# MuLabPKU/HD-PiSSA

Hardware: AMD Instinct MI355X
Metric: train tokens/sec (node) on the HD-PiSSA hot path, llama2-7b r16 (adapter probe fwd/bwd + Adam + dW aggregate + merge); dW merge+gather ms/step (higher is better)
Workload: dtype f32; 1 GPU; llama2-7b; model=llama2-7b, global_batch=16, seq_len=512, padding=per micro-batch to its longest sample (hp:190-201), micro_batches_per_rank=8, r_per_gpu=16, modules=224, exchange=gather, parallelism=dp1 (HD-PiSSA slices), x_layout=shared per projection group (q/k/v, gate/up)

## Files before the change

hd-pissa_amd/csrc/hdp_probe.hip:

```cpp
#include <chrono>
#include <cstdlib>
#include <cstring>
#include <mutex>
#include <vector>

#include "hdp_probe_int.h"

namespace hdp {

constexpr int kMaxGroup = 1024;
constexpr int kMaxSplit = 16;
constexpr int kP1Waves = 8;

static int p1_cols() {
  static const int v = [] { const char* e = getenv("HDP_P1_COLS"); return e ? atoi(e) : 128; }();
  return v;
}
static int p1_u() {
  static const int v = [] { const char* e = getenv("HDP_P1_U"); return e ? atoi(e) : 1; }();
  return v;
}
constexpr int kTC = 128;
constexpr int kNW = 256;

template <int CAP>
struct GroupArgsT {
  int n, rp, RB;
  int p1_pre[CAP + 1];
  int p2_pre[CAP + 1];
  int64_t p3_pre[CAP + 1];
  ProbeDesc d[CAP];
};
using GroupArgs = GroupArgsT<kMaxSplit>;
static_assert(sizeof(GroupArgs) <= 4096, "split-path kernel arguments must stay within 4 KB");

__device__ __forceinline__ int find_module(const int* pre, int n, int bid) {
  int m = 0;
  while (m + 1 < n && bid >= pre[m + 1]) ++m;
  return m;
}

template <bool F_RK>
__device__ __forceinline__ f32x4 load_f4(const float* F, int64_t K, int r, int j, int64_t k, int64_t k1, bool full) {
  f32x4 f;
  if (F_RK) {
    if (j < r && full) return *reinterpret_cast<const f32x4*>(F + (int64_t)j * K + k);
#pragma unroll
    for (int q = 0; q < 4; ++q) f[q] = (j < r && k + q < k1) ? F[(int64_t)j * K + k + q] : 0.f;
  } else {
#pragma unroll
    for (int q = 0; q < 4; ++q) f[q] = (j < r && k + q < k1) ? F[(k + q) * r + j] : 0.f;
  }
  return f;
}


template <int DT, int RB, int U, bool F_RK>
__device__ __forceinline__ void proj_wave(const void* Z, const float* F, int64_t T, int64_t K, int r, int64_t tb,
                                          int64_t k0, int64_t k1, int lane, float* tile, f32x4 (&acc)[RB]) {
// ... 308 lines not shown
}
__device__ __forceinline__ short bf16_bits(float v) { return (short)(__float_as_uint(v) >> 16); }
typedef __bf16 bf16x8 __attribute__((ext_vector_type(8)));
__device__ __forceinline__ void split8(const float (&v)[8], bf16x8& h, bf16x8& m, bf16x8& l) {
#pragma clang fp contract(off)
#pragma unroll
  for (int e = 0; e < 8; ++e) {
    const __bf16 a = (__bf16)v[e];
    const float r1 = v[e] - (float)a;
    const __bf16 b = (__bf16)r1;
    h[e] = a;
    m[e] = b;
    l[e] = (__bf16)(r1 - (float)b);
  }
}
__device__ __forceinline__ __bf16 as_bf16(float v) { return __builtin_bit_cast(__bf16, bf16_bits(v)); }
typedef uint32_t u32x4s __attribute__((ext_vector_type(4)));
__device__ __forceinline__ void split8p(const float (&v)[8], bf16x8& h, bf16x8& m, bf16x8& l) {
#pragma clang fp contract(off)
  u32x4s H, M, L;
#pragma unroll
  for (int e = 0; e < 4; ++e) {
    const float a0 = v[2 * e], a1 = v[2 * e + 1];
    const uint32_t ph = cvt_pk_bf16(a0, a1);
    const float r0 = a0 - __uint_as_float(ph << 16), r1 = a1 - __uint_as_float(ph & 0xffff0000u);
    const uint32_t pm = cvt_pk_bf16(r0, r1);
    const float s0 = r0 - __uint_as_float(pm << 16), s1 = r1 - __uint_as_float(pm & 0xffff0000u);
    H[e] = ph;
    M[e] = pm;
    L[e] = cvt_pk_bf16(s0, s1);
  }
  h = __builtin_bit_cast(bf16x8, H);
  m = __builtin_bit_cast(bf16x8, M);
  l = __builtin_bit_cast(bf16x8, L);
}
__device__ __forceinline__ f32x4 mfma_x6(const bf16x8 (&x)[3], const bf16x8 (&y)[3], f32x4 c) {
  c = __builtin_amdgcn_mfma_f32_16x16x32_bf16(x[1], y[1], c, 0, 0, 0);
  c = __builtin_amdgcn_mfma_f32_16x16x32_bf16(x[2], y[0], c, 0, 0, 0);
  c = __builtin_amdgcn_mfma_f32_16x16x32_bf16(x[0], y[2], c, 0, 0, 0);
  c = __builtin_amdgcn_mfma_f32_16x16x32_bf16(x[1], y[0], c, 0, 0, 0);
  c = __builtin_amdgcn_mfma_f32_16x16x32_bf16(x[0], y[1], c, 0, 0, 0);
  return __builtin_amdgcn_mfma_f32_16x16x32_bf16(x[0], y[0], c, 0, 0, 0);
}
__device__ __forceinline__ f32x4 mfma32(bf16x8 a, bf16x8 b, f32x4 c) {
  return __builtin_amdgcn_mfma_f32_16x16x32_bf16(a, b, c, 0, 0, 0);
}
__device__ __forceinline__ f32x4 mfma_bf16(bf16x4 a, bf16x4 b, f32x4 c) {
  return __builtin_amdgcn_mfma_f32_16x16x16bf16_1k(a, b, c, 0, 0, 0);
}

constexpr int kSwRedBufs = 4;
template <int RB, bool FUSE = false>
constexpr int sw_nbuf() { return FUSE ? 3 : RB >= 4 ? 2 : kSwRedBufs; }
#ifndef HDP_BF_SETS
#define HDP_BF_SETS 3
#endif
constexpr int kBfSets = HDP_BF_SETS;
enum { kSwProj = 1, kSwOuter = 2 };

template <int RB>
__device__ __forceinline__ void sw_store_g(const SweepDesc& d, const f32x4 (&acc2)[RB][4], int64_t col, int g,
                                           bool vec) {
#pragma clang fp contract(off)
  const float sc = d.scale;
  const int r = d.r;
  const int64_t N = d.N;
  if (!d.part_t) {
#pragma unroll
    for (int b = 0; b < RB; ++b)
#pragma unroll
      for (int reg = 0; reg < 4; ++reg) {
        const int j = 16 * b + 4 * g + reg;
        if (j >= r) continue;
        float* p = d.g + (int64_t)j * N + col;
        const f32x4 v{sc * acc2[b][0][reg], sc * acc2[b][1][reg], sc * acc2[b][2][reg], sc * acc2[b][3][reg]};
        if (vec) {
          gst4(p, d.acc ? gld4(p) + v : v);
        } else {
#pragma unroll
          for (int q = 0; q < 4; ++q)
            if (col + q < N) gst1(p + q, d.acc ? gld1(p + q) + v[q] : v[q]);
        }
      }
  } else {
    const bool v4 = (d.ldb & 3) == 0 && (reinterpret_cast<uintptr_t>(d.g) & 15) == 0;
#pragma unroll
    for (int b = 0; b < RB; ++b)
#pragma unroll
      for (int q = 0; q < 4; ++q) {
        if (col + q >= N) continue;
        const int j0 = 16 * b + 4 * g;
        float* p = d.g + (col + q) * d.ldb + j0;
        const f32x4 v = sc * acc2[b][q];
        if (v4 && j0 + 3 < r) {
          gst4(p, d.acc ? gld4(p) + v : v);
        } else {
#pragma unroll
          for (int reg = 0; reg < 4; ++reg)
            if (j0 + reg < r) gst1(p + reg, d.acc ? gld1(p + reg) + v[reg] : v[reg]);
        }
      }
  }
}

__device__ __forceinline__ void sw_store_g_fuse(const SweepDesc& d, const f32x4 (&acc2)[kSwMaxBlk][4], int64_t col,
                                                int g, bool vec) {
// ... 6 lines not shown
      const float sc = d.sc[b];
      const int acc = d.accb[b];
#pragma unroll
      for (int reg = 0; reg < 4; ++reg) {
        const int j = 4 * g + reg;
        if (j >= d.rbr[b]) continue;
        float* p = d.gb[b] + (int64_t)j * N + col;
        const f32x4 v{sc * acc2[b][0][reg], sc * acc2[b][1][reg], sc * acc2[b][2][reg], sc * acc2[b][3][reg]};
        if (vec) {
          gst4(p, acc ? gld4(p) + v : v);
        } else {
#pragma unroll
          for (int q = 0; q < 4; ++q)
            if (col + q < N) gst1(p + q, acc ? gld1(p + q) + v[q] : v[q]);
        }
      }
    }
  } else {
    const float sc = d.scale;
    const int r = d.r;
    const bool v4 = (d.ldb & 3) == 0 && (reinterpret_cast<uintptr_t>(d.g) & 15) == 0;
#pragma unroll
    for (int b = 0; b < kSwMaxBlk; ++b) {
      if (b >= d.nb) break;
#pragma unroll
      for (int q = 0; q < 4; ++q) {
        if (col + q >= N) continue;
        const int j0 = 16 * b + 4 * g;
        float* p = d.g + (col + q) * d.ldb + j0;
        const f32x4 v = sc * acc2[b][q];
        if (v4 && j0 + 3 < r) {
          gst4(p, d.acc ? gld4(p) + v : v);
        } else {
#pragma unroll
          for (int reg = 0; reg < 4; ++reg)
            if (j0 + reg < r) gst1(p + reg, d.acc ? gld1(p + reg) + v[reg] : v[reg]);
        }
      }
    }
  }
}

struct SweepArgs {
  int n, G;
  int spin;
  int64_t U;
  int* err;
  int* errd;
  const SweepDesc* d;
  const int* wst;
  const int* bnd;
};

template <int DT, int RB, int MODE, bool VEC, int OCC, bool FUSE, bool K32>
__device__ __forceinline__ void sweep_segment(const SweepDesc& d, int ct, int s0, int n, int64_t i0, int piece,
                                              const SweepArgs& sa, float* tile, float* red, int* flags, int wave,
                                              int lane) {
  constexpr bool PROJ = (MODE & kSwProj) != 0, OUTER = (MODE & kSwOuter) != 0;
  constexpr int rp = 16 * RB, r4 = rp / 4, ES = DT == HDP_F32 ? 4 : 2;
  const int li = lane & 15, g = lane >> 4;
  const int64_t T = d.T, N = d.N;
  const int64_t c = (int64_t)ct * kSwC + 64 * wave;
  const int64_t col = c + 4 * li;
  const int64_t colc = VEC ? (col < N ? col : N - 4) : col;
  const char* Zb = reinterpret_cast<const char*>(d.Z);

  constexpr bool SPLIT_F = DT == HDP_BF16 && MODE == kSwProj;
  constexpr bool X6 = K32 && DT == HDP_F32;
  constexpr bool K32P = K32 && MODE == kSwProj, K32O = K32 && MODE == kSwOuter;
  constexpr bool DL = K32P && DT == HDP_BF16 && !X6 && VEC;
  const int64_t cdl0 = c + 8 * g < N ? c + 8 * g : N - 8, cdl1 = c + 32 + 8 * g < N ? c + 32 + 8 * g : N - 8;
  f32x4 f[K32P ? 1 : 4][RB];
  bf16x4 fs[K32P ? 1 : 4][RB][3];
  bf16x8 fs8[K32P ? 2 : 1][RB][3];
  if constexpr (K32P) {
#pragma unroll
    for (int ch = 0; ch < 2; ++ch)
#pragma unroll
      for (int b = 0; b < RB; ++b) {
        const int j = 16 * b + li;
        const int64_t k = c + 32 * ch + 8 * g;
        float v[8];
#pragma unroll
        for (int e = 0; e < 8; ++e) v[e] = 0.f;
        const float* Fp = nullptr;
        int rows = d.r;
        if constexpr (FUSE) {
          Fp = b < d.nb ? d.Fb[b] : nullptr;
          rows = b < d.nb ? d.rbr[b] : 0;
        }
        const bool ok = FUSE ? (Fp != nullptr && li < rows) : (j < d.r);
        if (ok) {
          if (FUSE) Fp += (int64_t)li * N;
          if ((FUSE || d.f_rk) && N % 4 == 0 && k + 7 < N) {
            const float* P = FUSE ? Fp : d.F + (int64_t)j * N;
            const f32x4 a = gld4(P + k), bq = gld4(P + k + 4);
#pragma unroll
            for (int e = 0; e < 4; ++e) {
              v[e] = a[e];
              v[4 + e] = bq[e];
            }
          } else {
#pragma unroll
            for (int e = 0; e < 8; ++e)
              if (k + e < N)
                v[e] = FUSE ? gld1(Fp + k + e)
                            : d.f_rk ? gld1(d.F + (int64_t)j * N + k + e) : gld1(d.F + (k + e) * d.r + j);
          }
        }
        split8(v, fs8[ch][b][0], fs8[ch][b][1], fs8[ch][b][2]);
#pragma unroll
        for (int t = 0; t < 3; ++t) asm volatile("" : "+v"(fs8[ch][b][t]));
      }
  }
  if constexpr (PROJ && !K32P) {
#pragma unroll
    for (int s = 0; s < 4; ++s)
#pragma unroll
      for (int b = 0; b < RB; ++b) {
        const int j = 16 * b + li;
        const int64_t k = c + 16 * s + 4 * g;
        f32x4 v{0.f, 0.f, 0.f, 0.f};
        if constexpr (FUSE) {
          if (b < d.nb && li < d.rbr[b]) {
            const float* Fp = d.Fb[b] + (int64_t)li * N;
            if (N % 4 == 0 && k + 3 < N) {
              v = gld4(Fp + k);
            } else {
#pragma unroll
              for (int q = 0; q < 4; ++q)
                if (k + q < N) v[q] = gld1(Fp + k + q);
            }
          }
        } else if (j < d.r) {
          if (d.f_rk && N % 4 == 0 && k + 3 < N) {
            v = gld4(d.F + (int64_t)j * N + k);
          } else {
#pragma unroll
            for (int q = 0; q < 4; ++q)
              if (k + q < N) v[q] = d.f_rk ? gld1(d.F + (int64_t)j * N + k + q) : gld1(d.F + (k + q) * d.r + j);
          }
        }
        f[s][b] = v;
      }
    if constexpr (SPLIT_F) {
#pragma unroll
      for (int s = 0; s < 4; ++s)
#pragma unroll
        for (int b = 0; b < RB; ++b) {
          split3(f[s][b], fs[s][b][0], fs[s][b][1], fs[s][b][2]);
#pragma unroll
          for (int t = 0; t < 3; ++t) asm volatile("" : "+v"(fs[s][b][t]));
        }
    } else {
#pragma unroll
      for (int s = 0; s < 4; ++s)
#pragma unroll
        for (int b = 0; b < RB; ++b) asm volatile("" : "+v"(f[s][b]));
    }
  }
  bool hs_broken = false;
  f32x4 acc2[OUTER ? RB : 1][4];
#pragma unroll
  for (int b = 0; b < (OUTER ? RB : 1); ++b)
#pragma unroll
    for (int q = 0; q < 4; ++q) acc2[b][q] = f32x4{0.f, 0.f, 0.f, 0.f};

  constexpr bool DIST = PROJ && !FUSE && RB >= 4;
  int pend_i = -1, pend_s = 0;
  bool pend_tail = false;
  auto wait_ge = [&](const int* p, int target) {
    if (hs_broken) return;
    int it = 0;
    while (sa.spin < 0 || __hip_atomic_load(p, __ATOMIC_RELAXED, __HIP_MEMORY_SCOPE_WORKGROUP) < target) {
      if (it++ >= sa.spin) {
        hs_broken = true;
        if (lane == 0) {
          __hip_atomic_store(sa.err, 1, __ATOMIC_RELAXED, __HIP_MEMORY_SCOPE_SYSTEM);
          __hip_atomic_store(sa.errd, 1, __ATOMIC_RELAXED, __HIP_MEMORY_SCOPE_AGENT);
        }
        break;
      }
      __builtin_amdgcn_s_sleep(1);
    }
    asm volatile("" ::: "memory");
  };
  auto reduce_slice = [&](int pi, int ps, bool ptail) {
    if constexpr (DIST) {
      constexpr int NB = sw_nbuf<RB, FUSE>();
      const int pb = pi % NB, pr = pi / NB;
      wait_ge(flags + pb, kSwWaves * (pr + 1));
      const float* rs = red + pb * kSwWaves * 16 * rp;
      const int idx = 2 * lane;
      if (idx < 2 * rp) {
        const int row = 2 * wave + idx / rp, j = idx % rp;
        typedef float f32x2s __attribute__((ext_vector_type(2)));
        f32x2s acc{0.f, 0.f};
#pragma unroll
        for (int ww = 0; ww < kSwWaves; ++ww) acc += *reinterpret_cast<const f32x2s*>(rs + (ww * 16 + row) * rp + j);
        const int64_t t = 16 * (int64_t)ps + row;
        if (!ptail || t < T) *reinterpret_cast<HDP_GLOBAL f32x2s*>(gptr(d.slab_out + ((int64_t)ct * T + t) * rp + j)) = acc;
      }
      asm volatile("s_waitcnt lgkmcnt(0)" ::: "memory");
      if (lane == 0) (void)__hip_atomic_fetch_add(flags + NB + pb, 1, __ATOMIC_RELAXED, __HIP_MEMORY_SCOPE_WORKGROUP);
    }
  };

  auto compute = [&](const f32x4 (&z)[4], const float (&y)[4][RB], int s, int64_t i, bool tail) {
    if constexpr (OUTER) {
      if constexpr (DT == HDP_BF16) {
#pragma unroll
        for (int b = 0; b < RB; ++b) {
          if (FUSE && b >= d.nb) break;
          f32x4 yv;
#pragma unroll
          for (int p = 0; p < 4; ++p) yv[p] = (!tail || 16 * (int64_t)s + 4 * p + g < T) ? y[p][b] : 0.f;
          bf16x4 yh, ym, yl;
          split3(yv, yh, ym, yl);
#pragma unroll
          for (int q = 0; q < 4; ++q) {
            const bf16x4 zb{bf16_bits(z[0][q]), bf16_bits(z[1][q]), bf16_bits(z[2][q]), bf16_bits(z[3][q])};
            acc2[b][q] = mfma_bf16(yl, zb, acc2[b][q]);
            acc2[b][q] = mfma_bf16(ym, zb, acc2[b][q]);
            acc2[b][q] = mfma_bf16(yh, zb, acc2[b][q]);
          }
        }
      } else {
#pragma unroll
        for (int p = 0; p < 4; ++p) {
          const bool rok = !tail || 16 * (int64_t)s + 4 * p + g < T;
#pragma unroll
          for (int b = 0; b < RB; ++b) {
            if (FUSE && b >= d.nb) break;
            const float yv = rok ? y[p][b] : 0.f;
#pragma unroll
            for (int q = 0; q < 4; ++q) acc2[b][q] = __builtin_amdgcn_mfma_f32_16x16x4f32(yv, z[p][q], acc2[b][q], 0, 0, 0);
          }
        }
      }
    }
    if constexpr (PROJ) {
#pragma unroll
      for (int p = 0; p < (DL ? 0 : 4); ++p) *reinterpret_cast<f32x4*>(tile + (4 * p + g) * kTileLd + 4 * li) = z[p];
      f32x4 a0[RB], a1[RB];
#pragma unroll
      for (int b = 0; b < RB; ++b) a0[b] = a1[b] = f32x4{0.f, 0.f, 0.f, 0.f};
      if constexpr (K32P) {
#pragma unroll
        for (int ch = 0; ch < 2; ++ch) {
          f32x4 lo4{0.f, 0.f, 0.f, 0.f}, hi4{0.f, 0.f, 0.f, 0.f};
          if constexpr (!DL) {
            lo4 = *reinterpret_cast<const f32x4*>(tile + li * kTileLd + 32 * ch + 8 * g);
            hi4 = *reinterpret_cast<const f32x4*>(tile + li * kTileLd + 32 * ch + 8 * g + 4);
          }
          if constexpr (X6) {
            const float zv[8] = {lo4[0], lo4[1], lo4[2], lo4[3], hi4[0], hi4[1], hi4[2], hi4[3]};
            bf16x8 zs[3];
            split8p(zv, zs[0], zs[1], zs[2]);
#pragma unroll
            for (int b = 0; b < RB; ++b) {
              if (FUSE && b >= d.nb) break;
              f32x4& a = ch ? a1[b] : a0[b];
              a = mfma_x6(zs, fs8[ch][b], a);
            }
          } else {
            bf16x8 zb;
            if constexpr (DL) {
              zb = __builtin_bit_cast(bf16x8, z[ch]);
            } else {
#pragma unroll
              for (int e = 0; e < 4; ++e) {
                zb[e] = as_bf16(lo4[e]);
                zb[4 + e] = as_bf16(hi4[e]);
              }
            }
#pragma unroll
            for (int b = 0; b < RB; ++b) {
              if (FUSE && b >= d.nb) break;
              f32x4& a = ch ? a1[b] : a0[b];
              a = mfma32(zb, fs8[ch][b][2], a);
              a = mfma32(zb, fs8[ch][b][1], a);
              a = mfma32(zb, fs8[ch][b][0], a);
            }
          }
        }
      }
#pragma unroll
      for (int ss = 0; ss < (K32P ? 0 : 4); ++ss) {
        const f32x4 zf = *reinterpret_cast<const f32x4*>(tile + li * kTileLd + 16 * ss + 4 * g);
        if constexpr (SPLIT_F) {
          const bf16x4 zb{bf16_bits(zf[0]), bf16_bits(zf[1]), bf16_bits(zf[2]), bf16_bits(zf[3])};
#pragma unroll
          for (int b = 0; b < RB; ++b) {
            if (FUSE && b >= d.nb) break;
            f32x4& a = (ss & 1) ? a1[b] : a0[b];
            a = mfma_bf16(zb, fs[ss][b][2], a);
            a = mfma_bf16(zb, fs[ss][b][1], a);
            a = mfma_bf16(zb, fs[ss][b][0], a);
          }
        } else {
#pragma unroll
          for (int b = 0; b < RB; ++b) {
            if (FUSE && b >= d.nb) break;
#pragma unroll
            for (int q = 0; q < 4; ++q) {
              if (ss & 1) a1[b] = __builtin_amdgcn_mfma_f32_16x16x4f32(zf[q], f[ss][b][q], a1[b], 0, 0, 0);
              else a0[b] = __builtin_amdgcn_mfma_f32_16x16x4f32(zf[q], f[ss][b][q], a0[b], 0, 0, 0);
            }
          }
        }
      }
      HDP_MFMA_FENCE();
      constexpr int NBUF = sw_nbuf<RB, FUSE>();
      const int bsel = (int)(i % NBUF);
      const int round = (int)(i / NBUF);
      int* arrive = flags + bsel;
      int* done = flags + NBUF + bsel;
      if constexpr (DIST) {
        if (round > 0) wait_ge(done, kSwWaves * round);
        float* rb = red + (bsel * kSwWaves + wave) * 16 * rp;
#pragma unroll
        for (int b = 0; b < RB; ++b)
#pragma unroll
          for (int reg = 0; reg < 4; ++reg) rb[(4 * g + reg) * rp + 16 * b + li] = a0[b][reg] + a1[b][reg];
        asm volatile("s_waitcnt lgkmcnt(0)" ::: "memory");
        if (lane == 0) (void)__hip_atomic_fetch_add(arrive, 1, __ATOMIC_RELAXED, __HIP_MEMORY_SCOPE_WORKGROUP);
        if (pend_i >= 0) reduce_slice(pend_i, pend_s, pend_tail);
        pend_i = i;
        pend_s = s;
        pend_tail = tail;
      } else {
        if (round > 0 && !hs_broken) {
          int it = 0;
          while (sa.spin < 0 || __hip_atomic_load(done, __ATOMIC_RELAXED, __HIP_MEMORY_SCOPE_WORKGROUP) < round) {
            if (it++ >= sa.spin) {
              hs_broken = true;
              if (lane == 0) {
                __hip_atomic_store(sa.err, 1, __ATOMIC_RELAXED, __HIP_MEMORY_SCOPE_SYSTEM);
                __hip_atomic_store(sa.errd, 1, __ATOMIC_RELAXED, __HIP_MEMORY_SCOPE_AGENT);
              }
              break;
            }
            __builtin_amdgcn_s_sleep(1);
          }
          asm volatile("" ::: "memory");
        }
        float* rb = red + (bsel * kSwWaves + wave) * 16 * rp;
#pragma unroll
        for (int b = 0; b < RB; ++b) {
          if (FUSE && b >= d.nb) break;
#pragma unroll
          for (int reg = 0; reg < 4; ++reg) rb[(4 * g + reg) * rp + 16 * b + li] = a0[b][reg] + a1[b][reg];
        }
        asm volatile("s_waitcnt lgkmcnt(0)" ::: "memory");
        int old = 0;
        if (lane == 0) old = __hip_atomic_fetch_add(arrive, 1, __ATOMIC_RELAXED, __HIP_MEMORY_SCOPE_WORKGROUP);
        old = __builtin_amdgcn_readfirstlane(old);
        if (old == kSwWaves - 1) {
          asm volatile("s_waitcnt lgkmcnt(0)" ::: "memory");
          const float* rs = red + bsel * kSwWaves * 16 * rp;
          if constexpr (FUSE) {
#pragma unroll
            for (int b = 0; b < RB; ++b) {
              if (b >= d.nb) break;
              const int row = lane >> 2, jj = (lane & 3) * 4;
              f32x4 acc{0.f, 0.f, 0.f, 0.f};
#pragma unroll
              for (int ww = 0; ww < kSwWaves; ++ww)
                acc += *reinterpret_cast<const f32x4*>(rs + (ww * 16 + row) * rp + 16 * b + jj);
              const int64_t t = 16 * (int64_t)s + row;
              if (!tail || t < T) gst4(d.slab_b[b] + ((int64_t)ct * T + t) * d.rpm + jj, acc);
            }
          } else {
#pragma unroll
            for (int e0 = 0; e0 < 16 * r4; e0 += 64) {
              const int e = e0 + lane, row = e / r4, j = (e % r4) * 4;
              f32x4 acc{0.f, 0.f, 0.f, 0.f};
#pragma unroll
              for (int ww = 0; ww < kSwWaves; ++ww) acc += *reinterpret_cast<const f32x4*>(rs + (ww * 16 + row) * rp + j);
              const int64_t t = 16 * (int64_t)s + row;
              if (!tail || t < T) gst4(d.slab_out + ((int64_t)ct * T + t) * rp + j, acc);
            }
          }
          asm volatile("s_waitcnt lgkmcnt(0)" ::: "memory");
          if (lane == 0) {
            __hip_atomic_store(arrive, 0, __ATOMIC_RELAXED, __HIP_MEMORY_SCOPE_WORKGROUP);
            __hip_atomic_store(done, round + 1, __ATOMIC_RELAXED, __HIP_MEMORY_SCOPE_WORKGROUP);
          }
        }
      }
    }
  };

  auto pair = [&](const f32x4 (&zA)[4], const float (&yA)[4][RB], const f32x4 (&zB)[4], const float (&yB)[4][RB],
                  int s, bool vB, bool tail) {
    if constexpr (K32O && X6) {
      bf16x8 zs[4][3];
#pragma unroll
      for (int q = 0; q < 4; ++q) {
        const float zv[8] = {zA[0][q], zA[1][q], zA[2][q], zA[3][q],
                             vB ? zB[0][q] : 0.f, vB ? zB[1][q] : 0.f, vB ? zB[2][q] : 0.f, vB ? zB[3][q] : 0.f};
        split8p(zv, zs[q][0], zs[q][1], zs[q][2]);
      }
#pragma unroll
      for (int b = 0; b < RB; ++b) {
        if (FUSE && b >= d.nb) break;
        float yv[8];
#pragma unroll
        for (int p = 0; p < 4; ++p) {
          yv[p] = (!tail || 16 * (int64_t)s + 4 * p + g < T) ? yA[p][b] : 0.f;
          yv[4 + p] = vB ? yB[p][b] : 0.f;
        }
        bf16x8 ys[3];
        split8p(yv, ys[0], ys[1], ys[2]);
#pragma unroll
        for (int q = 0; q < 4; ++q) acc2[b][q] = mfma_x6(ys, zs[q], acc2[b][q]);
      }
    } else if constexpr (K32O) {
      bf16x8 zq[4];
#pragma unroll
      for (int q = 0; q < 4; ++q)
#pragma unroll
        for (int p = 0; p < 4; ++p) {
          zq[q][p] = as_bf16(zA[p][q]);
          zq[q][4 + p] = as_bf16(zB[p][q]);
        }
#pragma unroll
      for (int b = 0; b < RB; ++b) {
        if (FUSE && b >= d.nb) break;
        float yv[8];
#pragma unroll
        for (int p = 0; p < 4; ++p) {
          yv[p] = (!tail || 16 * (int64_t)s + 4 * p + g < T) ? yA[p][b] : 0.f;
          yv[4 + p] = vB ? yB[p][b] : 0.f;
        }
        bf16x8 yh, ym, yl;
        split8(yv, yh, ym, yl);
#pragma unroll
        for (int q = 0; q < 4; ++q) {
          acc2[b][q] = mfma32(yl, zq[q], acc2[b][q]);
          acc2[b][q] = mfma32(ym, zq[q], acc2[b][q]);
          acc2[b][q] = mfma32(yh, zq[q], acc2[b][q]);
        }
      }
    }
  };

  const int full_end = (int)min((int64_t)(s0 + n), T / 16);
  const int nfull = full_end > s0 ? full_end - s0 : 0;
  if (nfull > 0) {
    int64_t zo[4];
    int yo[4];
#pragma unroll
    for (int p = 0; p < 4; ++p) {
      zo[p] = ((16 * (int64_t)s0 + 4 * p + g) * N + colc) * ES;
      yo[p] = (16 * s0 + 4 * p + g) * d.yrs + li * d.yls;
    }
    const int64_t zstep = 16 * N * ES;
    int64_t zd = (16 * (int64_t)s0 + li) * N * ES;
    int lk = 0;
    auto load = [&](f32x4 (&z)[4], float (&y)[4][RB]) {
      __builtin_amdgcn_sched_barrier(0);
      if constexpr (DL) {
        typedef uint32_t u32x4d __attribute__((ext_vector_type(4)));
        z[0] = __builtin_bit_cast(f32x4, *reinterpret_cast<const HDP_GLOBAL u32x4d*>(gptr(Zb + zd + cdl0 * ES)));
        z[1] = __builtin_bit_cast(f32x4, *reinterpret_cast<const HDP_GLOBAL u32x4d*>(gptr(Zb + zd + cdl1 * ES)));
      }
#pragma unroll
      for (int p = 0; p < (DL ? 0 : 4); ++p) {
        if constexpr (VEC) {
          if constexpr (DT == HDP_F32)
            z[p] = load4_nt<DT>(Zb + zo[p], 0);
          else
            z[p] = load4<DT>(Zb + zo[p], 0);
        } else {
          const int64_t rowoff = zo[p] / ES - colc;
#pragma unroll
          for (int q = 0; q < 4; ++q) z[p][q] = load1<DT>(d.Z, rowoff + (col + q < N ? col + q : N - 1));
        }
        if constexpr (OUTER) {
          if constexpr (RB == 4) {
            const f32x4 v = gld4(d.y_in + yo[p]);
#pragma unroll
            for (int b = 0; b < RB; ++b) y[p][b] = v[b];
          } else if constexpr (RB == 2) {
            typedef float f32x2 __attribute__((ext_vector_type(2)));
            const f32x2 v = *reinterpret_cast<const HDP_GLOBAL f32x2*>(gptr(d.y_in + yo[p]));
            y[p][0] = v[0];
            y[p][1] = v[1];
          } else {
#pragma unroll
            for (int b = 0; b < RB; ++b) y[p][b] = gld1(d.y_in + yo[p] + b);
          }
        }
      }
      __builtin_amdgcn_sched_barrier(0);
      if (lk + 1 < nfull) {
        ++lk;
        zd += zstep;
#pragma unroll
        for (int p = 0; p < 4; ++p) {
          zo[p] += zstep;
// ... 22 lines not shown
      for (int j = 0; j + 1 < NS; ++j) load(zz[j], yy[j]);
      for (int k = 0; k < nfull; k += NS) {
#pragma unroll
        for (int j = 0; j < NS; ++j) {
          load(zz[(j + NS - 1) % NS], yy[(j + NS - 1) % NS]);
          if (j == 0 || k + j < nfull) compute(zz[j], yy[j], s0 + k + j, i0 + k + j, false);
        }
      }
    } else {
      f32x4 z0[4], z1[4];
      float y0[4][RB], y1[4][RB];
      load(z0, y0);
      for (int k = 0; k < nfull; k += 2) {
        load(z1, y1);
        compute(z0, y0, s0 + k, i0 + k, false);
        load(z0, y0);
        if (k + 1 < nfull) compute(z1, y1, s0 + k + 1, i0 + k + 1, false);
      }
    }
  }
  if (nfull < n) {
    const int s = s0 + nfull;
    f32x4 z[4];
    float y[4][RB];
    if constexpr (DL) {
      typedef uint32_t u32x4d __attribute__((ext_vector_type(4)));
      int64_t row = 16 * (int64_t)s + li;
      row = row < T ? row : T - 1;
      z[0] = __builtin_bit_cast(f32x4, *reinterpret_cast<const HDP_GLOBAL u32x4d*>(gptr(Zb + (row * N + cdl0) * ES)));
      z[1] = __builtin_bit_cast(f32x4, *reinterpret_cast<const HDP_GLOBAL u32x4d*>(gptr(Zb + (row * N + cdl1) * ES)));
    }
#pragma unroll
    for (int p = 0; p < (DL ? 0 : 4); ++p) {
      int64_t row = 16 * (int64_t)s + 4 * p + g;
      row = row < T ? row : T - 1;
      if constexpr (VEC) {
        z[p] = load4<DT>(d.Z, row * N + colc);
      } else {
#pragma unroll
        for (int q = 0; q < 4; ++q) z[p][q] = load1<DT>(d.Z, row * N + (col + q < N ? col + q : N - 1));
      }
      if constexpr (OUTER) {
#pragma unroll
        for (int b = 0; b < RB; ++b) y[p][b] = gld1(d.y_in + row * d.yrs + li * d.yls + b);
      }
    }
    if constexpr (K32O)
      pair(z, y, z, y, s, false, true);
    else
      compute(z, y, s, i0 + nfull, true);
  }
  if constexpr (DIST) {
    if (pend_i >= 0) reduce_slice(pend_i, pend_s, pend_tail);
  }
  if constexpr (OUTER) {
    HDP_MFMA_FENCE();
    if (s0 == 0 && n == d.S) {
      if constexpr (FUSE) {
        if (col < N) sw_store_g_fuse(d, acc2, col, g, VEC);
      } else {
        if (col < N) sw_store_g<RB>(d, acc2, col, g, VEC);
      }
    } else if (FUSE && col < N) {
      const int64_t pofs = ((int64_t)ct * d.kmax + piece) * d.rpm * kSwC;
#pragma unroll
      for (int b = 0; b < RB; ++b) {
        if (b >= d.nb) break;
        float* base = d.part_b[b] + pofs;
        if (!d.part_t) {
#pragma unroll
          for (int reg = 0; reg < 4; ++reg)
            gst4(base + (4 * g + reg) * kSwC + 64 * wave + 4 * li,
                 f32x4{acc2[b][0][reg], acc2[b][1][reg], acc2[b][2][reg], acc2[b][3][reg]});
        } else {
#pragma unroll
          for (int q = 0; q < 4; ++q) gst4(base + (64 * wave + 4 * li + q) * d.rpm + 4 * g, acc2[b][q]);
        }
      }
    } else if (col < N) {
      float* base = d.part + ((int64_t)ct * d.kmax + piece) * rp * kSwC;
      if (!d.part_t) {
#pragma unroll
        for (int b = 0; b < RB; ++b)
#pragma unroll
          for (int reg = 0; reg < 4; ++reg)
            gst4(base + (16 * b + 4 * g + reg) * kSwC + 64 * wave + 4 * li,
                 f32x4{acc2[b][0][reg], acc2[b][1][reg], acc2[b][2][reg], acc2[b][3][reg]});
      } else {
#pragma unroll
        for (int b = 0; b < RB; ++b)
#pragma unroll
          for (int q = 0; q < 4; ++q)
            gst4(base + (64 * wave + 4 * li + q) * rp + 16 * b + 4 * g, acc2[b][q]);
      }
    }
  }
}

template <int DT, int RB, int MODE, bool VEC, int OCC, bool FUSE = false, bool K32 = false>
__global__ __launch_bounds__(512, OCC == 2 ? 4 : 2) void probe_sweep_kernel(SweepArgs sa) {
  extern __shared__ __attribute__((aligned(16))) float lds[];
  const int w = blockIdx.x;
  const int64_t nsteps = sa.bnd[w + 1] - sa.bnd[w];
  if (nsteps <= 0) return;
  const int lane = threadIdx.x & 63, wave = threadIdx.x >> 6;
  float* tile = lds + wave * 16 * kTileLd;
  float* red = lds + kSwWaves * 16 * kTileLd;
  int* flags = reinterpret_cast<int*>(red + sw_nbuf<RB, FUSE>() * kSwWaves * 16 * 16 * RB);
  if constexpr ((MODE & kSwProj) != 0) {
    if (threadIdx.x < 2 * sw_nbuf<RB, FUSE>()) flags[threadIdx.x] = 0;
    __syncthreads();
  }
  int m = sa.wst[4 * w], ct = sa.wst[4 * w + 1], s = sa.wst[4 * w + 2];
  int piece = sa.wst[4 * w + 3];
  for (int64_t done = 0; done < nsteps;) {
    const SweepDesc d = sa.d[m];
    const int n = (int)min((int64_t)(d.S - s), nsteps - done);
    sweep_segment<DT, RB, MODE, VEC, OCC, FUSE, K32>(d, ct, s, n, done, piece, sa, tile, red, flags, wave, lane);
    done += n;
    s = 0;
    piece = 0;
    if (++ct == d.nct) {
      ct = 0;
      ++m;
    }
  }
}

struct YReduceArgs {
  int n, rp;
  const YRedDesc* d;
};

__global__ __launch_bounds__(256) void probe_yreduce_kernel(YReduceArgs ya) {
  const YRedDesc d = ya.d[blockIdx.y];
  const int64_t f = (int64_t)blockIdx.x * 256 + threadIdx.x;
  const int64_t step4 = d.T * ya.rp / 4;
  if (f >= step4) return;
  const f32x4* src = reinterpret_cast<const f32x4*>(d.slab) + f;
  f32x4 acc{0.f, 0.f, 0.f, 0.f};
  for (int c0 = 0; c0 < d.nct; c0 += 8) {
    f32x4 v[8];
#pragma unroll
    for (int u = 0; u < 8; ++u) v[u] = c0 + u < d.nct ? gld4(reinterpret_cast<const float*>(src + (c0 + u) * step4)) : f32x4{0.f, 0.f, 0.f, 0.f};
#pragma unroll
    for (int u = 0; u < 8; ++u) acc += v[u];
  }
  const int rp = ya.rp;
  const int64_t e = 4 * f, t = e / rp;
  const int j0 = (int)(e % rp), b = j0 / 16, li0 = j0 % 16;
  float* dst = d.y + t * d.ys + b;
#pragma unroll
  for (int k = 0; k < 4; ++k) gst1(dst + (li0 + k) * d.sl, acc[k]);
}

struct SwFinishArgs {
  int n, rp;
  const FinDesc* d;
  const int* jobs;
  int bx;
};

template <int V>
__global__ __launch_bounds__(256) void probe_sweep_finish_kernel(SwFinishArgs fa) {
#pragma clang fp contract(off)
  typedef float vec __attribute__((ext_vector_type(V)));
  const int job = blockIdx.x / fa.bx;
  const FinDesc& dm = fa.d[fa.jobs[4 * job]];
  const int code = fa.jobs[4 * job + 1], ct = code >> 1;
  const bool sideA = (code & 1) == 0;
  const int r = dm.r;
// ... 192 lines not shown
    switch (p1_u()) {
      case 1: hipLaunchKernelGGL((probe_proj_kernel<DT, RB, 1>), g1, b1, lds1(1), st, ga); break;
      case 3: hipLaunchKernelGGL((probe_proj_kernel<DT, RB, 3>), g1, b1, lds1(3), st, ga); break;
      default: hipLaunchKernelGGL((probe_proj_kernel<DT, RB, 2>), g1, b1, lds1(2), st, ga); break;
    }
  }
  }
  HDP_CHECK_LAUNCH();
  {
    KTimer kt(K_PROBE_P2, st, w.xg, w.fl_x + w.fl_g);
    hipLaunchKernelGGL((probe_outer_kernel<DT, RB>), dim3(ga.p2_pre[ga.n]), dim3(512),
                       (size_t)(kTC * rp > 4096 ? kTC * rp : 4096) * sizeof(float), st, ga);
  }
  HDP_CHECK_LAUNCH();
  const int64_t tot = ga.p3_pre[ga.n];
  const int blocks = (int)min((int64_t)4096, (tot + 255) / 256);
  bool v4 = true;
  int64_t per = 1;
  for (int i = 0; i < ga.n; ++i) {
    const ProbeDesc& d = ga.d[i];
    v4 = v4 && d.r % 4 == 0 && d.in % 4 == 0 && (reinterpret_cast<uintptr_t>(d.gA) & 15) == 0 &&
         (reinterpret_cast<uintptr_t>(d.gB) & 15) == 0 && (reinterpret_cast<uintptr_t>(d.partA) & 15) == 0 &&
         (reinterpret_cast<uintptr_t>(d.partB) & 15) == 0;
    const int64_t e = ((int64_t)d.r * (d.in + d.out) + 1023) / 1024;
    per = e > per ? e : per;
  }
  {
    KTimer kt(K_PROBE_FINISH, st, w.grads);
    if (v4 && per < 65536)
      hipLaunchKernelGGL(probe_finish4_kernel, dim3((unsigned)per, (unsigned)ga.n), dim3(256), 0, st, ga);
    else
      hipLaunchKernelGGL(probe_finish_kernel, dim3(blocks), dim3(256), 0, st, ga);
  }
  HDP_CHECK_LAUNCH();
  return HDP_OK;
}

struct SweepKernel {
  void (*fn)(SweepArgs);
  size_t lds;
};

static SweepKnobs sweep_knobs() {
  auto on = [](const char* name) {
    const char* e = getenv(name);
    return !(e && e[0] == '0');
  };
  SweepKnobs kn;
  kn.share_x = on("HDP_PROBE_SHARE_X");
  kn.balance = on("HDP_PROBE_BALANCE");
  const char* e = getenv("HDP_PROBE_K32");
  kn.k32 = !e ? 2 : e[0] == '0' ? 0 : e[0] == '4' ? 1 : e[0] == 'a' ? 3 : 2;
  kn.x6 = on("HDP_PROBE_X6");
  return kn;
}

template <int DT, int RB, bool VEC>
static void pick_sweep(bool fuse, const SweepKnobs& kn, SweepKernel (&pk)[3]) {
  constexpr int rp = 16 * RB;
  constexpr bool BF = DT == HDP_BF16;
  constexpr bool SPLIT_B = RB >= 4 && BF;
  constexpr size_t proj_lds =
      ((size_t)kSwWaves * 16 * kTileLd + (size_t)sw_nbuf<RB>() * kSwWaves * 16 * rp) * sizeof(float) +
      2 * sw_nbuf<RB>() * 4;
  constexpr size_t fuse_lds =
      ((size_t)kSwWaves * 16 * kTileLd + (size_t)sw_nbuf<kSwMaxBlk, true>() * kSwWaves * 16 * 16 * kSwMaxBlk) *
          sizeof(float) +
      2 * sw_nbuf<kSwMaxBlk, true>() * 4;
  constexpr int OCC_B = SPLIT_B ? 1 : RB >= 4 ? 3 : VEC ? 2 : 1;
  constexpr int MODE_B = SPLIT_B ? kSwProj : kSwProj | kSwOuter;
  constexpr bool CAN_FUSE = RB <= 2;
  constexpr int RBF = CAN_FUSE ? kSwMaxBlk : RB;
  const int k32m = BF ? kn.k32 : 0;
  const bool k32 = k32m >= 2 || (k32m == 1 && RB >= 4);
  const bool k32c = k32m == 3 || (k32m >= 1 && RB >= 4);
  const bool x6 = !BF && fuse && kn.x6;
  const bool kf = k32 || x6;
  const bool fused = CAN_FUSE && fuse;
  constexpr bool K32B = BF && MODE_B == kSwProj;
  if (fused) {
    if constexpr (CAN_FUSE)
      pk[0] = {kf ? probe_sweep_kernel<DT, RBF, kSwProj, VEC, 1, true, true>
                  : probe_sweep_kernel<DT, RBF, kSwProj, VEC, 1, true>,
               fuse_lds};
  } else {
    pk[0] = {k32 ? probe_sweep_kernel<DT, RB, kSwProj, VEC, 1, false, BF> : probe_sweep_kernel<DT, RB, kSwProj, VEC, 1>,
             proj_lds};
  }
  pk[1] = {k32 ? probe_sweep_kernel<DT, RB, MODE_B, VEC, OCC_B, false, K32B>
               : probe_sweep_kernel<DT, RB, MODE_B, VEC, OCC_B>,
           proj_lds};
  if (fused) {
    if constexpr (CAN_FUSE)
      pk[2] = {k32 ? probe_sweep_kernel<DT, RBF, kSwOuter, VEC, 1, true, BF>
                   : probe_sweep_kernel<DT, RBF, kSwOuter, VEC, 1, true>,
               0};
  } else {
    pk[2] = {k32c ? probe_sweep_kernel<DT, RB, kSwOuter, VEC, 1, false, BF> : probe_sweep_kernel<DT, RB, kSwOuter, VEC, 1>,
             0};
  }
}

static int sweep_slots(const SweepKernel& k) {
  struct Entry {
    void (*fn)(SweepArgs);
    int dev, slots;
  };
  static std::mutex mu;
  static std::vector<Entry> cache;
  int dev = 0;
  if (hipGetDevice(&dev) != hipSuccess || dev < 0) dev = 0;
  std::lock_guard<std::mutex> lk(mu);
  for (const Entry& e : cache)
    if (e.fn == k.fn && e.dev == dev) return e.slots;
  int cus = 0, per = 0;
  if (hipDeviceGetAttribute(&cus, hipDeviceAttributeMultiprocessorCount, dev) != hipSuccess || cus <= 0) cus = 256;
  if (hipOccupancyMaxActiveBlocksPerMultiprocessor(&per, k.fn, 512, k.lds) != hipSuccess || per <= 0) per = 1;
  cache.push_back(Entry{k.fn, dev, cus * per});
  return cus * per;
}

template <int DT, int RB, bool VEC>
static int launch_sweep(const HostGroup& ga, char* tab, hipStream_t st) {
  constexpr int rp = 16 * RB;
  const int n = ga.n;
  const SweepKnobs kn = sweep_knobs();
  SweepSides s;
  plan_sweep_sides(ga, DT == HDP_BF16, kn, s);
  SweepKernel pk[3];
  pick_sweep<DT, RB, VEC>(s.fuse, kn, pk);
  const int slots[3] = {sweep_slots(pk[0]), sweep_slots(pk[1]), sweep_slots(pk[2])};
  SweepTables t;
  const SweepError pe = plan_sweep_tables(ga, s, slots, t);
  static_assert(kSweepEInval == HDP_EINVAL, "the planner's error code");
  if (pe.code != 0) {
    set_error("%s", pe.msg);
// ... 409 lines not shown
```

hd-pissa_amd/csrc/hdp_sweep_plan.h:

```cpp
#pragma once
#include <cstddef>
#include <cstdint>
#include <cstring>
#include <vector>

#include "hdp_probe_plan.h"

namespace hdp {

struct ProbeDesc {
  const void* X;
  const void* G;
  const float* A;
  const float* B;
  float* gA;
  float* gB;
  float* slabH;
  float* slabJ;
  float* partA;
  float* partB;
  float* yH;
  float* yJ;
  int64_t T, in, out;
  float scale;
// ... 81 lines not shown
  return (size_t)(((in + kSwC - 1) / kSwC + (out + kSwC - 1) / kSwC) * 16 + 255) / 256 * 256;
}

inline int sweep_kmax(int64_t T) { return (int)(((T + 15) / 16 + kSwMinSteps - 1) / kSwMinSteps) + 2; }

template <class Item>
inline size_t sweep_table_bytes(const Item* it, int n) {
  size_t b = kTableFixed + (size_t)n * kTablePerModule;
  for (int i = 0; i < n; ++i) b += finish_jobs_bytes(it[i].in, it[i].out);
  return b;
}

inline ModPlan plan_sweep_module(int64_t T, int64_t in, int64_t out, int r) {
  ModPlan p;
  const int RB = rb_of(r), rp = 16 * RB;
  size_t off = 0;
  auto take = [&](size_t n) { size_t o = off; off += (n * 4 + 255) / 256 * 256; return o; };
  p.ksh = (int)((in + kSwC - 1) / kSwC);
  p.ksj = (int)((out + kSwC - 1) / kSwC);
  p.colh = p.colj = 0;
  p.kst = sweep_kmax(T);
  const size_t T16 = (size_t)((T + 15) / 16) * 16;
  p.off_slabH = take((size_t)p.ksh * T16 * rp);
  p.off_slabJ = take((size_t)p.ksj * T16 * rp);
  p.off_partA = take((size_t)p.ksh * p.kst * rp * kSwC);
  p.off_partB = take((size_t)p.ksj * p.kst * rp * kSwC);
  const size_t yrow = RB <= 2 ? 64 : 2 * (size_t)rp;
  p.off_yH = take(T16 * yrow);
  p.off_yJ = take(T16 * yrow);
  p.area = off;
  p.bytes = off + kTablePerModule + kTableFixed + 256 + finish_jobs_bytes(in, out);
  return p;
}

inline void place_module(ProbeDesc& d, const ModPlan& p, char* area) {
  d.slabH = reinterpret_cast<float*>(area + p.off_slabH);
  d.slabJ = reinterpret_cast<float*>(area + p.off_slabJ);
  d.partA = reinterpret_cast<float*>(area + p.off_partA);
  d.partB = reinterpret_cast<float*>(area + p.off_partB);
  d.yH = reinterpret_cast<float*>(area + p.off_yH);
  d.yJ = reinterpret_cast<float*>(area + p.off_yJ);
  d.ksh = p.ksh;
  d.ksj = p.ksj;
  d.kst = p.kst;
  d.colh = p.colh;
  d.colj = p.colj;
}

struct SweepKnobs {
  bool share_x = true;
  bool balance = true;
  int k32 = 2;
  bool x6 = true;
};

struct SweepError {
  int code;
  const char* msg;
};
constexpr int kSweepEInval = 1;

inline std::vector<std::vector<int>> shared_x_sets(const HostGroup& ga, bool share_x) {
  std::vector<std::vector<int>> sets;
  const int n = ga.n;
  if (ga.RB > 2 || !share_x) return sets;
  for (int i = 0; i < n; ++i)
    if (!ga.d[i].b_t) return sets;
  std::vector<char> used(n, 0);
  for (int i = 0; i < n; ++i) {
    if (used[i]) continue;
    const ProbeDesc& p = ga.d[i];
    std::vector<int> cur{i};
    int64_t outs = p.out;
    for (int k = i + 1; k < n && (int)(cur.size() + 1) * ga.RB <= kSwMaxBlk; ++k) {
      const ProbeDesc& q = ga.d[k];
      if (!used[k] && q.X == p.X && q.T == p.T && q.in == p.in) {
        cur.push_back(k);
        outs += q.out;
      }
    }
    if (cur.size() < 2 || outs < p.in) continue;
    for (int k : cur) used[k] = 1;
    sets.push_back(cur);
  }
  return sets;
}

inline SweepDesc side_desc(const ProbeDesc& p, bool xs, int RB, int S) {
  const int rp = 16 * RB;
  SweepDesc d{};
  d.Z = xs ? p.X : p.G;
  d.F = xs ? p.A : p.B;
  d.slab_out = xs ? p.slabH : p.slabJ;
  d.y_in = xs ? p.yJ : p.yH;
  d.part = xs ? p.partA : p.partB;
  d.T = p.T;
  d.N = xs ? p.in : p.out;
  d.pre = 0;
  d.r = p.r;
  d.f_rk = xs ? 1 : p.b_t;
  d.part_t = xs ? 0 : 1;
  d.nct = xs ? p.ksh : p.ksj;
  d.S = S;
  d.kmax = p.kst;
  d.g = xs ? p.gA : p.gB;
  d.scale = p.scale;
// ... 252 lines not shown
```

Before: 195,200 tokens/s.

## Replace last-arriver LDS reduction with claim-based cross-wave hand-off in fused probe sweep

```diff
diff --git a/hd-pissa_amd/csrc/hdp_handoff.h b/hd-pissa_amd/csrc/hdp_handoff.h
--- /dev/null
+++ b/hd-pissa_amd/csrc/hdp_handoff.h
@@ -0,0 +1,94 @@
+#pragma once
+#include <stdint.h>
+
+#if defined(__HIPCC__)
+#define HDP_HO __host__ __device__ __forceinline__
+#else
+#define HDP_HO inline
+#endif
+
+namespace hdp {
+
+constexpr int kHoWaves = 8;
+
+template <int NBUF, int UMAX>
+constexpr int ho_words() { return NBUF * (2 + UMAX); }
+template <int NBUF, class I>
+HDP_HO int ho_buf(I i) { return static_cast<int>(i % NBUF); }
+template <int NBUF, class I>
+HDP_HO int ho_round(I i) { return static_cast<int>(i / NBUF); }
+template <int NBUF>
+HDP_HO int ho_arrive_at(int b) { return b; }
+template <int NBUF>
+HDP_HO int ho_done_at(int b) { return NBUF + b; }
+template <int NBUF, int UMAX>
+HDP_HO int ho_claim_at(int b, int u) { return 2 * NBUF + b * UMAX + u; }
+
+HDP_HO bool ho_complete(int arrived, int ro) { return arrived >= kHoWaves * (ro + 1); }
+HDP_HO bool ho_may_write(int done, int ro, int units) { return done >= units * ro; }
+HDP_HO bool ho_done(int done, int ro, int units) { return done >= units * (ro + 1); }
+HDP_HO bool ho_claimable(int arrived, int claim, int ro) { return ho_complete(arrived, ro) && claim == ro; }
+
+template <int NBUF, class M, class I>
+HDP_HO void ho_arrive(M& m, typename M::Word* flags, I i) {
+  m.add(flags + ho_arrive_at<NBUF>(ho_buf<NBUF>(i)), 1);
+}
+
+template <int NBUF, int UMAX, class M, class I, class Sum>
+HDP_HO bool ho_take(M& m, typename M::Word* flags, I j, int u, Sum&& sum) {
+  const int b = ho_buf<NBUF>(j), ro = ho_round<NBUF>(j);
+  if (!m.cas(flags + ho_claim_at<NBUF, UMAX>(b, u), ro, ro + 1)) return false;
+  sum(j, u);
+  m.add(flags + ho_done_at<NBUF>(b), 1);
+  return true;
+}
+
+template <int NBUF, int UMAX, class M, class I, class Sum>
+HDP_HO void ho_look(M& m, typename M::Word* flags, I i, I i0, int units, Sum&& sum) {
+  if (i - 1 < i0) return;
+  const typename M::Snap s = m.snap(flags, ho_words<NBUF, UMAX>());
+#if defined(__HIPCC__)
+#pragma unroll
+#endif
+  for (int k = 1; k < NBUF; ++k) {
+    const I j = i - k;
+    if (j < i0) break;
+    const int b = ho_buf<NBUF>(j), ro = ho_round<NBUF>(j);
+    if (!ho_complete(m.get(s, ho_arrive_at<NBUF>(b)), ro)) continue;
+    for (int u = 0; u < units; ++u)
+      if (m.get(s, ho_claim_at<NBUF, UMAX>(b, u)) == ro) ho_take<NBUF, UMAX>(m, flags, j, u, sum);
+  }
+}
+
+template <int NBUF, int UMAX, class M, class I, class Sum>
+HDP_HO bool ho_settle(M& m, typename M::Word* flags, I j, int units, int spin, Sum&& sum) {
+  const int b = ho_buf<NBUF>(j), ro = ho_round<NBUF>(j);
+  int it = 0;
+  for (;;) {
+    if (spin >= 0 && ho_done(m.load(flags + ho_done_at<NBUF>(b)), ro, units)) return true;
+    if (ho_complete(m.load(flags + ho_arrive_at<NBUF>(b)), ro)) {
+      bool took = false;
+      for (int u = 0; u < units; ++u)
+        if (m.load(flags + ho_claim_at<NBUF, UMAX>(b, u)) == ro) took = ho_take<NBUF, UMAX>(m, flags, j, u, sum) || took;
+      if (took && spin >= 0) continue;
+    }
+    if (it++ >= spin) return false;
+    m.pause();
+  }
+}
+
+template <int NBUF, int UMAX, class M, class I, class Sum>
+HDP_HO bool ho_acquire(M& m, typename M::Word* flags, I i, I i0, int units, int spin, Sum&& sum) {
+  if (i - NBUF < i0) return true;
+  return ho_settle<NBUF, UMAX>(m, flags, i - NBUF, units, spin, sum);
+}
+
+template <int NBUF, int UMAX, class M, class I, class Sum>
+HDP_HO bool ho_flush(M& m, typename M::Word* flags, I i0, int n, int units, int spin, Sum&& sum) {
+  const I end = i0 + n;
+  for (I j = end - NBUF < i0 ? i0 : end - NBUF; j < end; ++j)
+    if (!ho_settle<NBUF, UMAX>(m, flags, j, units, spin, sum)) return false;
+  return true;
+}
+
+}
diff --git a/hd-pissa_amd/csrc/hdp_probe.hip b/hd-pissa_amd/csrc/hdp_probe.hip
--- a/hd-pissa_amd/csrc/hdp_probe.hip
+++ b/hd-pissa_amd/csrc/hdp_probe.hip
@@ -2,9 +2,11 @@
 #include <cstdlib>
 #include <cstring>
 #include <mutex>
+#include <type_traits>
 #include <vector>
 
 #include "hdp_probe_int.h"
+#include "hdp_handoff.h"
 
 namespace hdp {
 
@@ -419,6 +421,36 @@
 constexpr int kSwRedBufs = 4;
 template <int RB, bool FUSE = false>
 constexpr int sw_nbuf() { return FUSE ? 3 : RB >= 4 ? 2 : kSwRedBufs; }
+struct LdsHandoff {
+  typedef int Word;
+  typedef int Snap;
+  int lane;
+  __device__ __forceinline__ int load(const int* p) const {
+    return __builtin_amdgcn_readfirstlane(__hip_atomic_load(p, __ATOMIC_RELAXED, __HIP_MEMORY_SCOPE_WORKGROUP));
+  }
+  __device__ __forceinline__ void add(int* p, int v) const {
+    if (lane == 0) (void)__hip_atomic_fetch_add(p, v, __ATOMIC_RELAXED, __HIP_MEMORY_SCOPE_WORKGROUP);
+  }
+  __device__ __forceinline__ bool cas(int* p, int expect, int desired) const {
+    int won = 0;
+    if (lane == 0)
+      won = __hip_atomic_compare_exchange_strong(p, &expect, desired, __ATOMIC_RELAXED, __ATOMIC_RELAXED,
+                                                 __HIP_MEMORY_SCOPE_WORKGROUP)
+                ? 1
+                : 0;
+    return __builtin_amdgcn_readfirstlane(won) != 0;
+  }
+  __device__ __forceinline__ void pause() const { __builtin_amdgcn_s_sleep(1); }
+  __device__ __forceinline__ Snap snap(const int* flags, int n) const {
+    int v = 0;
+    if (lane < n) v = __hip_atomic_load(flags + lane, __ATOMIC_RELAXED, __HIP_MEMORY_SCOPE_WORKGROUP);
+    return v;
+  }
+  __device__ __forceinline__ int get(const Snap& s, int k) const { return __builtin_amdgcn_readlane(s, k); }
+};
+static_assert(kHoWaves == kSwWaves, "the hand-off counts one partial per wave");
+template <int RB, bool FUSE = false>
+constexpr int sw_nflags(bool claim) { return claim ? ho_words<sw_nbuf<RB, FUSE>(), 1>() : 2 * sw_nbuf<RB, FUSE>(); }
 #ifndef HDP_BF_SETS
 #define HDP_BF_SETS 3
 #endif
@@ -531,7 +563,7 @@
   const int* bnd;
 };
 
-template <int DT, int RB, int MODE, bool VEC, int OCC, bool FUSE, bool K32>
+template <int DT, int RB, int MODE, bool VEC, int OCC, bool FUSE, bool K32, bool CLAIM>
 __device__ __forceinline__ void sweep_segment(const SweepDesc& d, int ct, int s0, int n, int64_t i0, int piece,
                                               const SweepArgs& sa, float* tile, float* red, int* flags, int wave,
                                               int lane) {
@@ -638,7 +670,16 @@
         for (int b = 0; b < RB; ++b) asm volatile("" : "+v"(f[s][b]));
     }
   }
+  const int full_end = (int)min((int64_t)(s0 + n), T / 16);
+  const int nfull = full_end > s0 ? full_end - s0 : 0;
   bool hs_broken = false;
+  auto report_broken = [&]() {
+    hs_broken = true;
+    if (lane == 0) {
+      __hip_atomic_store(sa.err, 1, __ATOMIC_RELAXED, __HIP_MEMORY_SCOPE_SYSTEM);
+      __hip_atomic_store(sa.errd, 1, __ATOMIC_RELAXED, __HIP_MEMORY_SCOPE_AGENT);
+    }
+  };
   f32x4 acc2[OUTER ? RB : 1][4];
 #pragma unroll
   for (int b = 0; b < (OUTER ? RB : 1); ++b)
@@ -653,11 +694,7 @@
     int it = 0;
     while (sa.spin < 0 || __hip_atomic_load(p, __ATOMIC_RELAXED, __HIP_MEMORY_SCOPE_WORKGROUP) < target) {
       if (it++ >= sa.spin) {
-        hs_broken = true;
-        if (lane == 0) {
-          __hip_atomic_store(sa.err, 1, __ATOMIC_RELAXED, __HIP_MEMORY_SCOPE_SYSTEM);
-          __hip_atomic_store(sa.errd, 1, __ATOMIC_RELAXED, __HIP_MEMORY_SCOPE_AGENT);
-        }
+        report_broken();
         break;
       }
       __builtin_amdgcn_s_sleep(1);
@@ -685,6 +722,45 @@
     }
   };
 
+  auto sum_step = [&](int bsel, int s, bool tail, auto fresh) {
+    if constexpr (PROJ && !DIST) {
+      int ln = lane;
+      if (fresh.value) asm volatile("" : "+v"(ln));
+      asm volatile("s_waitcnt lgkmcnt(0)" ::: "memory");
+      const float* rs = red + bsel * kSwWaves * 16 * rp;
+      if constexpr (FUSE) {
+#pragma unroll
+        for (int b = 0; b < RB; ++b) {
+          if (b >= d.nb) break;
+          const int row = ln >> 2, jj = (ln & 3) * 4;
+          f32x4 acc{0.f, 0.f, 0.f, 0.f};
+#pragma unroll
+          for (int ww = 0; ww < kSwWaves; ++ww)
+            acc += *reinterpret_cast<const f32x4*>(rs + (ww * 16 + row) * rp + 16 * b + jj);
+          const int64_t t = 16 * (int64_t)s + row;
+          if (!tail || t < T) gst4(d.slab_b[b] + ((int64_t)ct * T + t) * d.rpm + jj, acc);
+        }
+      } else {
+#pragma unroll
+        for (int e0 = 0; e0 < 16 * r4; e0 += 64) {
+          const int e = e0 + ln, row = e / r4, j = (e % r4) * 4;
+          f32x4 acc{0.f, 0.f, 0.f, 0.f};
+#pragma unroll
+          for (int ww = 0; ww < kSwWaves; ++ww) acc += *reinterpret_cast<const f32x4*>(rs + (ww * 16 + row) * rp + j);
+          const int64_t t = 16 * (int64_t)s + row;
+          if (!tail || t < T) gst4(d.slab_out + ((int64_t)ct * T + t) * rp + j, acc);
+        }
+      }
+      asm volatile("s_waitcnt lgkmcnt(0)" ::: "memory");
+    }
+  };
+  LdsHandoff hm{lane};
+  const int hi0 = (int)i0;
+  auto sum_claimed = [&](int j, int) {
+    const int k = j - hi0;
+    sum_step((int)(j % sw_nbuf<RB, FUSE>()), s0 + k, k >= nfull, std::true_type{});
+  };
+
   auto compute = [&](const f32x4 (&z)[4], const float (&y)[4][RB], int s, int64_t i, bool tail) {
     if constexpr (OUTER) {
       if constexpr (DT == HDP_BF16) {
@@ -721,6 +797,12 @@
     if constexpr (PROJ) {
 #pragma unroll
       for (int p = 0; p < (DL ? 0 : 4); ++p) *reinterpret_cast<f32x4*>(tile + (4 * p + g) * kTileLd + 4 * li) = z[p];
+      if constexpr (CLAIM && !DIST) {
+        if (!hs_broken &&
+            !ho_acquire<sw_nbuf<RB, FUSE>(), 1>(hm, flags, (int)i, hi0, 1, sa.spin, sum_claimed))
+          report_broken();
+        asm volatile("" ::: "memory");
+      }
       f32x4 a0[RB], a1[RB];
 #pragma unroll
       for (int b = 0; b < RB; ++b) a0[b] = a1[b] = f32x4{0.f, 0.f, 0.f, 0.f};
@@ -808,16 +890,23 @@
         pend_i = i;
         pend_s = s;
         pend_tail = tail;
+      } else if constexpr (CLAIM) {
+        float* rb = red + (bsel * kSwWaves + wave) * 16 * rp;
+#pragma unroll
+        for (int b = 0; b < RB; ++b) {
+          if (FUSE && b >= d.nb) break;
+#pragma unroll
+          for (int reg = 0; reg < 4; ++reg) rb[(4 * g + reg) * rp + 16 * b + li] = a0[b][reg] + a1[b][reg];
+        }
+        asm volatile("s_waitcnt lgkmcnt(0)" ::: "memory");
+        ho_arrive<NBUF>(hm, flags, (int)i);
+        ho_look<NBUF, 1>(hm, flags, (int)i, hi0, 1, sum_claimed);
       } else {
         if (round > 0 && !hs_broken) {
           int it = 0;
           while (sa.spin < 0 || __hip_atomic_load(done, __ATOMIC_RELAXED, __HIP_MEMORY_SCOPE_WORKGROUP) < round) {
             if (it++ >= sa.spin) {
-              hs_broken = true;
-              if (lane == 0) {
-                __hip_atomic_store(sa.err, 1, __ATOMIC_RELAXED, __HIP_MEMORY_SCOPE_SYSTEM);
-                __hip_atomic_store(sa.errd, 1, __ATOMIC_RELAXED, __HIP_MEMORY_SCOPE_AGENT);
-              }
+              report_broken();
               break;
             }
             __builtin_amdgcn_s_sleep(1);
@@ -836,32 +925,7 @@
         if (lane == 0) old = __hip_atomic_fetch_add(arrive, 1, __ATOMIC_RELAXED, __HIP_MEMORY_SCOPE_WORKGROUP);
         old = __builtin_amdgcn_readfirstlane(old);
         if (old == kSwWaves - 1) {
-          asm volatile("s_waitcnt lgkmcnt(0)" ::: "memory");
-          const float* rs = red + bsel * kSwWaves * 16 * rp;
-          if constexpr (FUSE) {
-#pragma unroll
-            for (int b = 0; b < RB; ++b) {
-              if (b >= d.nb) break;
-              const int row = lane >> 2, jj = (lane & 3) * 4;
-              f32x4 acc{0.f, 0.f, 0.f, 0.f};
-#pragma unroll
-              for (int ww = 0; ww < kSwWaves; ++ww)
-                acc += *reinterpret_cast<const f32x4*>(rs + (ww * 16 + row) * rp + 16 * b + jj);
-              const int64_t t = 16 * (int64_t)s + row;
-              if (!tail || t < T) gst4(d.slab_b[b] + ((int64_t)ct * T + t) * d.rpm + jj, acc);
-            }
-          } else {
-#pragma unroll
-            for (int e0 = 0; e0 < 16 * r4; e0 += 64) {
-              const int e = e0 + lane, row = e / r4, j = (e % r4) * 4;
-              f32x4 acc{0.f, 0.f, 0.f, 0.f};
-#pragma unroll
-              for (int ww = 0; ww < kSwWaves; ++ww) acc += *reinterpret_cast<const f32x4*>(rs + (ww * 16 + row) * rp + j);
-              const int64_t t = 16 * (int64_t)s + row;
-              if (!tail || t < T) gst4(d.slab_out + ((int64_t)ct * T + t) * rp + j, acc);
-            }
-          }
-          asm volatile("s_waitcnt lgkmcnt(0)" ::: "memory");
+          sum_step(bsel, s, tail, std::false_type{});
           if (lane == 0) {
             __hip_atomic_store(arrive, 0, __ATOMIC_RELAXED, __HIP_MEMORY_SCOPE_WORKGROUP);
             __hip_atomic_store(done, round + 1, __ATOMIC_RELAXED, __HIP_MEMORY_SCOPE_WORKGROUP);
@@ -925,8 +989,6 @@
     }
   };
 
-  const int full_end = (int)min((int64_t)(s0 + n), T / 16);
-  const int nfull = full_end > s0 ? full_end - s0 : 0;
   if (nfull > 0) {
     int64_t zo[4];
     int yo[4];
@@ -1055,6 +1117,9 @@
   }
   if constexpr (DIST) {
     if (pend_i >= 0) reduce_slice(pend_i, pend_s, pend_tail);
+  } else if constexpr (PROJ && CLAIM) {
+    if (!hs_broken && !ho_flush<sw_nbuf<RB, FUSE>(), 1>(hm, flags, hi0, n, 1, sa.spin, sum_claimed))
+      report_broken();
   }
   if constexpr (OUTER) {
     HDP_MFMA_FENCE();
@@ -1100,7 +1165,7 @@
   }
 }
 
-template <int DT, int RB, int MODE, bool VEC, int OCC, bool FUSE = false, bool K32 = false>
+template <int DT, int RB, int MODE, bool VEC, int OCC, bool FUSE = false, bool K32 = false, bool CLAIM = false>
 __global__ __launch_bounds__(512, OCC == 2 ? 4 : 2) void probe_sweep_kernel(SweepArgs sa) {
   extern __shared__ __attribute__((aligned(16))) float lds[];
   const int w = blockIdx.x;
@@ -1111,7 +1176,7 @@
   float* red = lds + kSwWaves * 16 * kTileLd;
   int* flags = reinterpret_cast<int*>(red + sw_nbuf<RB, FUSE>() * kSwWaves * 16 * 16 * RB);
   if constexpr ((MODE & kSwProj) != 0) {
-    if (threadIdx.x < 2 * sw_nbuf<RB, FUSE>()) flags[threadIdx.x] = 0;
+    if (threadIdx.x < sw_nflags<RB, FUSE>(CLAIM)) flags[threadIdx.x] = 0;
     __syncthreads();
   }
   int m = sa.wst[4 * w], ct = sa.wst[4 * w + 1], s = sa.wst[4 * w + 2];
@@ -1119,7 +1184,7 @@
   for (int64_t done = 0; done < nsteps;) {
     const SweepDesc d = sa.d[m];
     const int n = (int)min((int64_t)(d.S - s), nsteps - done);
-    sweep_segment<DT, RB, MODE, VEC, OCC, FUSE, K32>(d, ct, s, n, done, piece, sa, tile, red, flags, wave, lane);
+    sweep_segment<DT, RB, MODE, VEC, OCC, FUSE, K32, CLAIM>(d, ct, s, n, done, piece, sa, tile, red, flags, wave, lane);
     done += n;
     s = 0;
     piece = 0;
@@ -1418,6 +1483,8 @@
   const char* e = getenv("HDP_PROBE_K32");
   kn.k32 = !e ? 2 : e[0] == '0' ? 0 : e[0] == '4' ? 1 : e[0] == 'a' ? 3 : 2;
   kn.x6 = on("HDP_PROBE_X6");
+  e = getenv("HDP_PROBE_HANDOFF");
+  kn.handoff_last = e && strcmp(e, "last") == 0;
   return kn;
 }
 
@@ -1428,11 +1495,11 @@
   constexpr bool SPLIT_B = RB >= 4 && BF;
   constexpr size_t proj_lds =
       ((size_t)kSwWaves * 16 * kTileLd + (size_t)sw_nbuf<RB>() * kSwWaves * 16 * rp) * sizeof(float) +
-      2 * sw_nbuf<RB>() * 4;
+      sw_nflags<RB>(false) * 4;
   constexpr size_t fuse_lds =
       ((size_t)kSwWaves * 16 * kTileLd + (size_t)sw_nbuf<kSwMaxBlk, true>() * kSwWaves * 16 * 16 * kSwMaxBlk) *
           sizeof(float) +
-      2 * sw_nbuf<kSwMaxBlk, true>() * 4;
+      sw_nflags<kSwMaxBlk, true>(true) * 4;
   constexpr int OCC_B = SPLIT_B ? 1 : RB >= 4 ? 3 : VEC ? 2 : 1;
   constexpr int MODE_B = SPLIT_B ? kSwProj : kSwProj | kSwOuter;
   constexpr bool CAN_FUSE = RB <= 2;
@@ -1446,8 +1513,10 @@
   constexpr bool K32B = BF && MODE_B == kSwProj;
   if (fused) {
     if constexpr (CAN_FUSE)
-      pk[0] = {kf ? probe_sweep_kernel<DT, RBF, kSwProj, VEC, 1, true, true>
-                  : probe_sweep_kernel<DT, RBF, kSwProj, VEC, 1, true>,
+      pk[0] = {kn.handoff_last ? (kf ? probe_sweep_kernel<DT, RBF, kSwProj, VEC, 1, true, true>
+                                     : probe_sweep_kernel<DT, RBF, kSwProj, VEC, 1, true>)
+                               : (kf ? probe_sweep_kernel<DT, RBF, kSwProj, VEC, 1, true, true, true>
+                                     : probe_sweep_kernel<DT, RBF, kSwProj, VEC, 1, true, false, true>),
                fuse_lds};
   } else {
     pk[0] = {k32 ? probe_sweep_kernel<DT, RB, kSwProj, VEC, 1, false, BF> : probe_sweep_kernel<DT, RB, kSwProj, VEC, 1>,
diff --git a/hd-pissa_amd/csrc/hdp_sweep_plan.h b/hd-pissa_amd/csrc/hdp_sweep_plan.h
--- a/hd-pissa_amd/csrc/hdp_sweep_plan.h
+++ b/hd-pissa_amd/csrc/hdp_sweep_plan.h
@@ -157,6 +157,7 @@
   bool balance = true;
   int k32 = 2;
   bool x6 = true;
+  bool handoff_last = false;
 };
 
 struct SweepError {
```

Result: no change. 194,800 tokens/s (median of 2 runs) (-0.2%).
